# qq456cvb/CPPF2

Measured on AMD Instinct MI355X. Metric: scenes/sec (1/2/4/8 GPU) at 4096 pts x 20k tuples; 5deg5cm match vs ref, higher is better.
Workload: dtype f32

## Files before the change

### cppf2_amd/csrc/cppf_mlp_split.hip

```cpp
#include "cppf_common.h"
#include <atomic>
#include <mutex>
#include <type_traits>

typedef float f32x16 __attribute__((ext_vector_type(16)));
typedef float f32x4 __attribute__((ext_vector_type(4)));
typedef __bf16 bf16x8 __attribute__((ext_vector_type(8)));

__host__ __device__ constexpr int rs_waves(int nt) { return nt >= 6 ? 4 : 8; }
#define RS_RESLAYER 0
#define RS_LINEAR 1
#define RS_SUMGATHER 2
#define RS_ENCODE 3
#define RS_SUMENCODE 5
__host__ __device__ constexpr int rs_waves_mode(int nt, int mode) { return mode == RS_LINEAR ? 8 : rs_waves(nt); }
__host__ __device__ constexpr int rs_stage_tiles(int mode) { return 16; }
__host__ __device__ constexpr int rs_wgs_per_cu(int mode) { return 1; }
#define RS_FRAG_BYTES 1024
__host__ __device__ constexpr int rs_stage_bytes(int stg) { return stg * 3 * RS_FRAG_BYTES; }
__host__ __device__ constexpr int rs_tile_bytes(int pc) { return pc * RS_FRAG_BYTES; }

#ifndef RS_DEEP_PREFETCH
#define RS_DEEP_PREFETCH 0
#endif
// ... 325 lines not shown
};

template <int NT, int PC>
__device__ __forceinline__ void rs_decode_epilogue(f32x16 (&o)[NT], const RsDecode& dc, int64_t row, bool in, int g, float bs) {
  static_assert(NT == 6, "6 coordinates x 32 bins");
  if (PC == 2) {
#pragma unroll
    for (int u = 0; u < 6; ++u) o[u] *= bs;
  }
  if (dc.prior) {
    const float* pr = dc.prior + row * 192 + 4 * g;
#pragma unroll
    for (int u = 0; u < 6; ++u) {
#pragma unroll
      for (int q = 0; q < 4; ++q) {
        const f32x4 v = *reinterpret_cast<const f32x4*>(pr + 32 * u + 8 * q);
        o[u][4 * q + 0] += v.x; o[u][4 * q + 1] += v.y; o[u][4 * q + 2] += v.z; o[u][4 * q + 3] += v.w;
      }
    }
  } else if (dc.prior_pos) {
    const float* pp = dc.prior_pos + row * 6;
    const float is = dc.prior_inv_sigma;
#pragma unroll
    for (int u = 0; u < 6; ++u) {
      const float pos = pp[u];
#pragma unroll
      for (int e = 0; e < 16; ++e) {
        const float z = ((float)((e & 3) + 8 * (e >> 2) + 4 * g) - pos) * is;
        o[u][e] += (z * z) * -0.5f;
      }
    }
  }
  float back[6], tot[6];
#pragma unroll
  for (int u = 0; u < 6; ++u) {
    float m = o[u][0];
#pragma unroll
    for (int e = 1; e < 16; ++e) m = fmaxf(m, o[u][e]);
    m = fmaxf(m, __shfl_xor(m, 32));
#pragma unroll
    for (int e = 0; e < 16; ++e) o[u][e] = softmax_exp(o[u][e] - m);
    back[u] = 0.0f;
  }
#pragma unroll
  for (int q = 0; q < 4; ++q) {
    float ta[6][4], tb[6][4], fwd[6];
#pragma unroll
    for (int u = 0; u < 6; ++u) {
      ta[u][0] = back[u] + o[u][4 * q + 0];
      ta[u][1] = ta[u][0] + o[u][4 * q + 1];
      ta[u][2] = ta[u][1] + o[u][4 * q + 2];
      ta[u][3] = ta[u][2] + o[u][4 * q + 3];
    }
#pragma unroll
    for (int u = 0; u < 6; ++u) fwd[u] = __shfl_xor(ta[u][3], 32);
#pragma unroll
    for (int u = 0; u < 6; ++u) {
      tb[u][0] = fwd[u] + o[u][4 * q + 0];
      tb[u][1] = tb[u][0] + o[u][4 * q + 1];
      tb[u][2] = tb[u][1] + o[u][4 * q + 2];
      tb[u][3] = tb[u][2] + o[u][4 * q + 3];
    }
#pragma unroll
    for (int u = 0; u < 6; ++u) {
      back[u] = __shfl_xor(tb[u][3], 32);
      tot[u] = g ? tb[u][3] : back[u];
#pragma unroll
      for (int i = 0; i < 4; ++i) o[u][4 * q + i] = g ? tb[u][i] : ta[u][i];
    }
  }
  const float* ur = dc.uniforms + row * 6;
#pragma unroll
  for (int u = 0; u < 6; ++u) {
    const float target = ur[u] * tot[u];
    int cnt = 0;
#pragma unroll
    for (int e = 0; e < 16; ++e) cnt += (o[u][e] <= target) ? 1 : 0;
    cnt += __shfl_xor(cnt, 32);
    if (in && g == 0) dc.bins[row * 6 + u] = cnt < 31 ? cnt : 31;
  }
}

__device__ __forceinline__ void rs_claim_store(int* p, int v) { __hip_atomic_store(p, v, __ATOMIC_RELAXED, __HIP_MEMORY_SCOPE_WORKGROUP); }
__device__ __forceinline__ int rs_claim_load(int* p) { return __hip_atomic_load(p, __ATOMIC_RELAXED, __HIP_MEMORY_SCOPE_WORKGROUP); }

struct RsTap {
  float* out = nullptr;
  int64_t ld = 0;
};

struct RsGather {
  const int32_t* gidx = nullptr;
  const float* table = nullptr;
  int slots = 0, head = 0, fshift = 0;
  int64_t tld = 0;
  const float* pts = nullptr;
  const float* nrm = nullptr;
  const int32_t* pt_off = nullptr;
  const int32_t* tup_off = nullptr;
  int B = 0;
  int* sched = nullptr;
};

struct RsRow3 {
  float x, y, z;
};

__device__ __forceinline__ void rs_encode_tiles(char* slots, int lane, int g, const float* __restrict__ pts, const float* __restrict__ nrm,
                                                const float* __restrict__ table, int fshift, int g0, int g1, int g2, int g3, int g4) {
  constexpr int PI_[10] = {0, 0, 0, 0, 1, 1, 1, 2, 2, 3}, PJ_[10] = {1, 2, 3, 4, 2, 3, 4, 3, 4, 4};
  const int gi[5] = {g0, g1, g2, g3, g4};
  float v[48];
  {
    float p[5][3];
#pragma unroll
    for (int q = 0; q < 5; ++q) {
      const RsRow3 r = *reinterpret_cast<const RsRow3*>(pts + 3 * (int64_t)gi[q]);
      p[q][0] = r.x; p[q][1] = r.y; p[q][2] = r.z;
    }
#pragma unroll
    for (int q = 0; q < 10; ++q)
#pragma unroll
      for (int c = 0; c < 3; ++c) v[3 * q + c] = p[PI_[q]][c] - p[PJ_[q]][c];
  }
  {
    float n[5][3];
#pragma unroll
    for (int q = 0; q < 5; ++q) {
      const RsRow3 r = *reinterpret_cast<const RsRow3*>(nrm + 3 * (int64_t)gi[q]);
      n[q][0] = r.x; n[q][1] = r.y; n[q][2] = r.z;
    }
#pragma unroll
    for (int q = 0; q < 10; ++q) {
      const float* ni = n[PI_[q]];
      const float* nj = n[PJ_[q]];
      const float s_ = (ni[0] * nj[0] + ni[1] * nj[1]) + ni[2] * nj[2];
      v[30 + q] = fmaxf(s_, -s_);
    }
  }
  {
    const float* d0 = table + ((int64_t)g0 << fshift);
    const f32x4 a = *reinterpret_cast<const f32x4*>(d0), b = *reinterpret_cast<const f32x4*>(d0 + 4);
    v[40] = a.x; v[41] = a.y; v[42] = a.z; v[43] = a.w; v[44] = b.x; v[45] = b.y; v[46] = b.z; v[47] = b.w;
  }
#pragma unroll
  for (int s = 0; s < 3; ++s) {
    f32x4 lo, hi;
    lo.x = g ? v[16 * s + 8] : v[16 * s + 0]; lo.y = g ? v[16 * s + 9] : v[16 * s + 1];
    lo.z = g ? v[16 * s + 10] : v[16 * s + 2]; lo.w = g ? v[16 * s + 11] : v[16 * s + 3];
    hi.x = g ? v[16 * s + 12] : v[16 * s + 4]; hi.y = g ? v[16 * s + 13] : v[16 * s + 5];
    hi.z = g ? v[16 * s + 14] : v[16 * s + 6]; hi.w = g ? v[16 * s + 15] : v[16 * s + 7];
    *reinterpret_cast<f32x4*>(slots + s * 2048 + lane * 16) = lo;
    *reinterpret_cast<f32x4*>(slots + s * 2048 + 1024 + lane * 16) = hi;
  }
}

__device__ __forceinline__ void rs_encode_coord_tiles(char* slots, int lane, int g, const float* __restrict__ pts, int g0, int g1, int g2,
                                                      int g3, int g4) {
  constexpr int PI_[10] = {0, 0, 0, 0, 1, 1, 1, 2, 2, 3}, PJ_[10] = {1, 2, 3, 4, 2, 3, 4, 3, 4, 4};
  const int gi[5] = {g0, g1, g2, g3, g4};
  float p[5][3], v[32];
#pragma unroll
  for (int q = 0; q < 5; ++q) {
    const RsRow3 r = *reinterpret_cast<const RsRow3*>(pts + 3 * (int64_t)gi[q]);
    p[q][0] = r.x; p[q][1] = r.y; p[q][2] = r.z;
  }
#pragma unroll
  for (int q = 0; q < 10; ++q)
#pragma unroll
    for (int c = 0; c < 3; ++c) v[3 * q + c] = p[PI_[q]][c] - p[PJ_[q]][c];
  v[30] = 0.0f; v[31] = 0.0f;
#pragma unroll
  for (int s = 0; s < 2; ++s) {
    f32x4 lo, hi;
    lo.x = g ? v[16 * s + 8] : v[16 * s + 0]; lo.y = g ? v[16 * s + 9] : v[16 * s + 1];
    lo.z = g ? v[16 * s + 10] : v[16 * s + 2]; lo.w = g ? v[16 * s + 11] : v[16 * s + 3];
    hi.x = g ? v[16 * s + 12] : v[16 * s + 4]; hi.y = g ? v[16 * s + 13] : v[16 * s + 5];
    hi.z = g ? v[16 * s + 14] : v[16 * s + 6]; hi.w = g ? v[16 * s + 15] : v[16 * s + 7];
    *reinterpret_cast<f32x4*>(slots + s * 2048 + lane * 16) = lo;
    *reinterpret_cast<f32x4*>(slots + s * 2048 + 1024 + lane * 16) = hi;
  }
}

template <int NT, bool PROJ, bool GATHER, bool DECODE = false, int PC = 3, int MODE = RS_RESLAYER>
__global__ __launch_bounds__(64 * rs_waves_mode(NT, MODE), rs_wgs_per_cu(MODE)) void reslayer_split_kernel(const float* x, int64_t ldx, int k_in, float* out,
                                                                              int64_t ldo, int64_t rows,
                                                                              const char* __restrict__ wq,
                                                                              const float* __restrict__ b1,
                                                                              const float* __restrict__ b0, int chain,
                                                                              RsGather ga, RsDecode dc, RsTap tap, float wscale) {
  const float bs = (PC == 2) ? 1.0f / wscale : 1.0f;
  constexpr int WAVES = rs_waves_mode(NT, MODE), THREADS = 64 * WAVES, BLOCK_ROWS = 32 * WAVES;
  constexpr int T0 = PROJ ? 2 * NT : NT;
  constexpr bool LIN = MODE == RS_LINEAR;
  static_assert(!LIN || (!PROJ && !GATHER && !DECODE), "a plain Linear has one product");
  constexpr bool SUMG = MODE == RS_SUMGATHER || MODE == RS_SUMENCODE;
  constexpr bool LOCAL_IDX = MODE == RS_ENCODE || MODE == RS_SUMENCODE;
  static_assert(!SUMG || (PROJ && !GATHER), "the table sums stand for columns of a projection layer's input");
  static_assert(MODE != RS_ENCODE || (GATHER && !DECODE), "RS_ENCODE is a form of the gathering launch");
  constexpr bool PF = RS_DEEP_PREFETCH && WAVES == 4;
  extern __shared__ __attribute__((aligned(16))) char s_ring[];
  const int lane = threadIdx.x & 63;
  const int wave = __builtin_amdgcn_readfirstlane(threadIdx.x >> 6);
  const int r = lane & 31, g = lane >> 5;
  const int ks1 = (k_in + 15) >> 4;
  const int64_t nblocks = (rows + BLOCK_ROWS - 1) / BLOCK_ROWS;
  int64_t bfirst = blockIdx.x, bstride = gridDim.x, bend = nblocks;
  if (RS_XCD_BLOCKS && (gridDim.x & 7) == 0 && nblocks >= 64) {
    const int64_t xcd = blockIdx.x & 7;
    bfirst = nblocks * xcd / 8 + (blockIdx.x >> 3);
    bend = nblocks * (xcd + 1) / 8;
    bstride = gridDim.x >> 3;
  }
  int* const sched = ga.sched;
  const bool dyn = sched != nullptr && !LIN;
  int* const s_claim = reinterpret_cast<int*>(s_ring + 2 * rs_stage_bytes(rs_stage_tiles(MODE)) + WAVES * 3 * 2048 + (2 + chain) * 32 * NT * 4);
  if (dyn) { bfirst = blockIdx.x; bstride = 0; bend = nblocks; }
  const int64_t mine = dyn ? (bfirst < bend ? 1 : 0) : (bend > bfirst ? (bend - bfirst + bstride - 1) / bstride : 0);
  if (dyn && threadIdx.x == 0) rs_claim_store(&s_claim[0], (int)gridDim.x + atomicAdd(&sched[0], 1));

  constexpr int STG = rs_stage_tiles(MODE), RING_BYTES = 2 * rs_stage_bytes(STG);
  RsStream<NT, T0, WAVES, PC, LIN, STG> ws;
  const int64_t seg_bytes = (int64_t)ks1 * T0 * rs_tile_bytes(PC);
  if (LIN) {
    wq += (int64_t)blockIdx.y * chain * seg_bytes;
    b1 = b1 ? b1 + (int64_t)blockIdx.y * chain * 32 * NT : b1;
    out += (int64_t)blockIdx.y * chain * 32 * NT;
  }
  ws.base = wq;
  ws.ring = s_ring;
  ws.ks1 = ks1;
  ws.seg = 0;
  ws.pos = 0;
  ws.off = 0;
  ws.shape(chain);
  ws.left = mine * ws.chunks;
  ws.stage = 0;
  ws.wave = wave;
  ws.lane = lane;
  ws.prime();
  float* s_b1 = reinterpret_cast<float*>(s_ring + RING_BYTES + WAVES * 3 * 2048);
  float* s_b0 = s_b1 + 32 * NT;
  if (LIN) {
    for (int i = threadIdx.x; i < 32 * NT * chain; i += THREADS) s_b1[i] = b1 ? b1[i] : 0.0f;
  } else {
    for (int i = threadIdx.x; i < 32 * NT; i += THREADS) {
      s_b1[i] = b1[i];
      if (PROJ) s_b0[i] = b0[i];
    }
    for (int i = threadIdx.x; i < 32 * NT * chain; i += THREADS) s_b1[2 * 32 * NT + i] = b1[32 * NT + i];
  }
  __syncthreads();

  RsX<GATHER> xs;
  xs.slots = s_ring + RING_BYTES + wave * (3 * 2048);
  xs.k_in = k_in;
  xs.g = g;
  xs.lane = lane;
  xs.table = ga.table;
  xs.head = ga.head;
  xs.fshift = ga.fshift;
  auto row_of = [&](int64_t blk) {
    const int64_t row = blk * BLOCK_ROWS + wave * 32 + r;
    const int64_t rc = row < rows ? row : rows - 1;
    RsRow rw;
    rw.xrow = LOCAL_IDX ? ga.table : x + rc * ldx;
    rw.g0 = rw.g1 = rw.g2 = rw.g3 = rw.g4 = rw.g5 = rw.g6 = rw.g7 = 0;
    if (GATHER || SUMG) {
      const int32_t* p = ga.gidx + rc * ga.slots;
      int p0 = 0;
      if (LOCAL_IDX) {
        int lo = 0, hi = ga.B;
        while (hi - lo > 1) {
          const int mid = (lo + hi) >> 1;
          if ((int64_t)ga.tup_off[mid] <= rc) lo = mid; else hi = mid;
        }
        p0 = ga.pt_off[lo];
      }
      rw.g0 = p[0];
      rw.g1 = ga.slots > 1 ? p[1] : 0; rw.g2 = ga.slots > 2 ? p[2] : 0; rw.g3 = ga.slots > 3 ? p[3] : 0;
      rw.g4 = ga.slots > 4 ? p[4] : 0; rw.g5 = ga.slots > 5 ? p[5] : 0; rw.g6 = ga.slots > 6 ? p[6] : 0;
      rw.g7 = ga.slots > 7 ? p[7] : 0;
      if (LOCAL_IDX) {
        rw.g0 += p0; rw.g1 += ga.slots > 1 ? p0 : 0; rw.g2 += ga.slots > 2 ? p0 : 0; rw.g3 += ga.slots > 3 ? p0 : 0;
        rw.g4 += ga.slots > 4 ? p0 : 0; rw.g5 += ga.slots > 5 ? p0 : 0; rw.g6 += ga.slots > 6 ? p0 : 0; rw.g7 += ga.slots > 7 ? p0 : 0;
      }
    }
    return rw;
  };
  int64_t next_blk = dyn ? (int64_t)rs_claim_load(&s_claim[0]) : bfirst + bstride;
  int par = 1;
  RsRow cur = row_of(bfirst < bend ? bfirst : 0);
  auto first_tiles = [&](const RsRow rw) {
    if constexpr (MODE == RS_ENCODE) {
      rs_encode_tiles(xs.slots, lane, g, ga.pts, ga.nrm, ga.table, ga.fshift, rw.g0, rw.g1, rw.g2, rw.g3, rw.g4);
    } else if constexpr (MODE == RS_SUMENCODE) {
      rs_encode_coord_tiles(xs.slots, lane, g, ga.pts, rw.g0, rw.g1, rw.g2, rw.g3, rw.g4);
    } else {
      xs.issue(0, 0, rw);
      xs.issue(1, 1, rw);
      xs.issue(2, 2, rw);
    }
  };
  if (bfirst < bend) first_tiles(cur);
  if constexpr (LIN) {
    for (int64_t blk = bfirst; blk < bend; blk += bstride) {
      const int64_t row = blk * BLOCK_ROWS + wave * 32 + r;
      const bool in = row < rows;
      const bool more = blk + bstride < bend;
      const RsRow nxt = row_of(more ? blk + bstride : blk);
#pragma unroll 1
      for (int grp = 0; grp < chain; ++grp) {
        f32x16 acc[NT];
#pragma unroll
        for (int u = 0; u < NT; ++u) rs_load_tile(acc[u], s_b1 + 32 * (grp * NT + u), g);
        rs_product_x<NT, false, PC>(acc, xs, cur, ks1, ws);
        const bool last = grp + 1 == chain;
        if (!last || more) {
          const RsRow nx = last ? nxt : cur;
          xs.issue(0, 0, nx);
          xs.issue(1, 1, nx);
          xs.issue(2, 2, nx);
        }
        if (in) {
          float* orow = out + row * ldo + (int64_t)grp * 32 * NT + 4 * g;
#pragma unroll
          for (int u = 0; u < NT; ++u) {
#pragma unroll
            for (int q = 0; q < 4; ++q) {
              f32x4 v;
              v.x = acc[u][4 * q + 0]; v.y = acc[u][4 * q + 1]; v.z = acc[u][4 * q + 2]; v.w = acc[u][4 * q + 3];
              if (PC == 2) v *= bs;
              *reinterpret_cast<f32x4*>(orow + 32 * u + 8 * q) = v;
            }
          }
        }
      }
      cur = nxt;
    }
    RS_WAIT(0, 15);
    return;
  }
  for (int64_t blk = bfirst; blk < bend;) {
    const int64_t row = blk * BLOCK_ROWS + wave * 32 + r;
    const bool in = row < rows;
    const float* xrow = cur.xrow;
    const int64_t nb = dyn ? next_blk : blk + bstride;
    const bool more = nb < bend;
    if (dyn && more) ws.left += ws.chunks;
    const RsRow nxt = row_of(more ? nb : blk);
    int claim = 0;
    if (dyn && threadIdx.x == 0) claim = atomicAdd(&sched[0], 1);
    f32x16 acc[2 * NT];
    f32x16 (&h)[NT] = *reinterpret_cast<f32x16 (*)[NT]>(&acc[0]);
    f32x16 (&o)[NT] = *reinterpret_cast<f32x16 (*)[NT]>(&acc[NT]);
#pragma unroll
    for (int u = 0; u < T0; ++u) rs_load_tile(acc[u], s_b1 + 32 * u, g);
    if constexpr (SUMG) {
#pragma unroll 1
      for (int i = 0; i < ((RS_DBG & 64) ? 0 : ga.slots); ++i) {
        int p = cur.g0;
        p = i == 1 ? cur.g1 : p; p = i == 2 ? cur.g2 : p; p = i == 3 ? cur.g3 : p; p = i == 4 ? cur.g4 : p;
        p = i == 5 ? cur.g5 : p; p = i == 6 ? cur.g6 : p; p = i == 7 ? cur.g7 : p;
        if (RS_DBG & 128) p &= 255;
        const float* trow = ga.table + ((int64_t)p * ga.tld + (int64_t)i * (32 * T0)) + 4 * g;
#pragma unroll
        for (int u0 = 0; u0 < T0; u0 += 4) {
          f32x4 t[16];
#pragma unroll
          for (int j = 0; j < 16; ++j) t[j] = *reinterpret_cast<const f32x4*>(trow + 32 * (u0 + (j >> 2)) + 8 * (j & 3));
#pragma unroll
          for (int j = 0; j < 16; ++j) {
            f32x16& a = acc[u0 + (j >> 2)];
            const int q = j & 3;
            if (PC == 2) {
              a[4 * q + 0] += t[j].x * wscale; a[4 * q + 1] += t[j].y * wscale; a[4 * q + 2] += t[j].z * wscale; a[4 * q + 3] += t[j].w * wscale;
            } else {
              a[4 * q + 0] += t[j].x; a[4 * q + 1] += t[j].y; a[4 * q + 2] += t[j].z; a[4 * q + 3] += t[j].w;
            }
          }
        }
      }
    }
    if (!PROJ && (WAVES == 8 || RS_EARLY_RESIDUAL)) {
#pragma unroll
      for (int u = 0; u < NT; ++u) {
        if (PC == 2) rs_load_tile_scaled(o[u], ((RS_DBG & 32) ? (const float*)s_b1 : xrow) + 32 * u, g, wscale);
        else rs_load_tile(o[u], ((RS_DBG & 32) ? (const float*)s_b1 : xrow) + 32 * u, g);
      }
    }
    {
      f32x16 (&first)[T0] = *reinterpret_cast<f32x16 (*)[T0]>(&acc[0]);
      rs_product_x<T0, PF, PC>(first, xs, cur, ks1, ws);
    }
#pragma unroll
    for (int u = 0; u < NT; ++u) {
#pragma unroll
      for (int e = 0; e < 16; ++e) h[u][e] = (h[u][e] < 0.0f) ? 0.0f : h[u][e];
    }
    if (!PROJ && WAVES == 4 && !RS_EARLY_RESIDUAL) {
      if (PC == 2) {
#pragma unroll
        for (int u = 0; u < NT; u += 2) {
          rs_load_tile_scaled(o[u], ((RS_DBG & 32) ? (const float*)s_b1 : xrow) + 32 * u, g, wscale);
          if (u + 1 < NT) rs_load_tile_scaled(o[u + 1], ((RS_DBG & 32) ? (const float*)s_b1 : xrow) + 32 * (u + 1), g, wscale);
#pragma unroll
          for (int e = 0; e < 16; ++e) {
            asm volatile("" : "+a"(o[u][e]));
            if (u + 1 < NT) asm volatile("" : "+a"(o[u + 1][e]));
          }
          __builtin_amdgcn_sched_barrier(0);
        }
      } else {
#pragma unroll
        for (int u = 0; u < NT; ++u) rs_load_tile(o[u], ((RS_DBG & 32) ? (const float*)s_b1 : xrow) + 32 * u, g);
      }
    }
    if (dyn && threadIdx.x == 0) rs_claim_store(&s_claim[par], (int)gridDim.x + claim);
    if (more) first_tiles(nxt);
    cur = nxt;
    rs_product_h<NT, NT, PF, PC>(o, h, ws, bs);
    if (tap.out && in) {
      float* trow = tap.out + row * tap.ld + 4 * g;
#pragma unroll
      for (int u = 0; u < NT; ++u) {
#pragma unroll
        for (int q = 0; q < 4; ++q) {
          f32x4 v;
          v.x = o[u][4 * q + 0]; v.y = o[u][4 * q + 1]; v.z = o[u][4 * q + 2]; v.w = o[u][4 * q + 3];
          if (PC == 2) v *= bs;
          *reinterpret_cast<f32x4*>(trow + 32 * u + 8 * q) = v;
        }
      }
    }
#pragma unroll 1
    for (int l = 0; l < chain; ++l) {
      const float* bl = s_b1 + 32 * NT * (2 + l);
#pragma unroll
      for (int u = 0; u < NT; ++u) rs_load_tile(h[u], bl + 32 * u, g);
      rs_product_h<NT, NT, PF, PC>(h, o, ws, bs);
#pragma unroll
      for (int u = 0; u < NT; ++u) {
#pragma unroll
        for (int e = 0; e < 16; ++e) h[u][e] = (h[u][e] < 0.0f) ? 0.0f : h[u][e];
      }
      rs_product_h<NT, NT, PF, PC>(o, h, ws, bs);
    }
    if (DECODE) {
      if constexpr (NT == 6) rs_decode_epilogue<NT, PC>(o, dc, in ? row : rows - 1, in, g, bs);
    } else if (in && (!(RS_DBG & 32) || o[0][0] == 1.2345e30f)) {
      float* orow = out + row * ldo + 4 * g;
#pragma unroll
      for (int u = 0; u < NT; ++u) {
#pragma unroll
        for (int q = 0; q < 4; ++q) {
          f32x4 v;
          v.x = o[u][4 * q + 0]; v.y = o[u][4 * q + 1]; v.z = o[u][4 * q + 2]; v.w = o[u][4 * q + 3];
          if (PC == 2) v *= bs;
          *reinterpret_cast<f32x4*>(orow + 32 * u + 8 * q) = v;
        }
      }
    }
    blk = nb;
    if (dyn) {
      next_blk = rs_claim_load(&s_claim[par]);
      par ^= 1;
    }
  }
  RS_WAIT(0, 15);
  if (dyn && threadIdx.x == 0) {
    if (atomicAdd(&sched[1], 1) == (int)gridDim.x - 1) {
      __hip_atomic_store(&sched[0], 0, __ATOMIC_RELAXED, __HIP_MEMORY_SCOPE_AGENT);
      __hip_atomic_store(&sched[1], 0, __ATOMIC_RELAXED, __HIP_MEMORY_SCOPE_AGENT);
    }
  }
}

static int64_t rs_stream_bytes(int32_t k_in, int32_t n_out, int32_t proj, int32_t chain, int pc) {
  if (k_in <= 0 || !(n_out == 64 || n_out == 128 || n_out == 192 || n_out == 256) || chain < 0 || chain > 15) return -1;
  const int64_t nt = n_out / 32, ks1 = (k_in + 15) / 16;
  return (ks1 * (proj ? 2 : 1) + (1 + 2 * (int64_t)chain) * 2 * nt) * nt * rs_tile_bytes(pc);
}

extern "C" int64_t cppf_reslayer_split_stream_bytes(int32_t k_in, int32_t n_out, int32_t proj, int32_t chain) {
  return rs_stream_bytes(k_in, n_out, proj, chain, 3);
}

static std::atomic<int> g_rs_debug_cus{0};
extern "C" int cppf_reslayer_split_debug_grid(int32_t workgroups) {
  g_rs_debug_cus.store(workgroups > 0 ? workgroups : 0);
  return CPPF_OK;
}

static std::atomic<int> g_rs_reserved_cus{0};
extern "C" int cppf_mlp_reserve_cus(int32_t cus) {
  CPPF_CHECK_ARG(cus <= 1024);
  return cus < 0 ? g_rs_reserved_cus.load() : g_rs_reserved_cus.exchange(cus);
}

template <int NT, bool PROJ, bool GATHER = false, bool DECODE = false, int PC = 3, int MODE = RS_RESLAYER>
static int rs_launch(const float* x, int64_t ldx, int k_in, float* out, int64_t ldo, int64_t rows, const char* wq,
                     const float* b1, const float* b0, int chain, int cus, hipStream_t stream, RsGather ga = RsGather(),
                     RsDecode dc = RsDecode(), RsTap tap = RsTap(), float wscale = 1.0f) {
  constexpr int WAVES = rs_waves_mode(NT, MODE), THREADS = 64 * WAVES, BLOCK_ROWS = 32 * WAVES;
  const int64_t nblocks = (rows + BLOCK_ROWS - 1) / BLOCK_ROWS;
  const int forced = g_rs_debug_cus.load();
  if (forced > 0) cus = forced;
  else cus = cus - g_rs_reserved_cus.load() > cus / 2 ? cus - g_rs_reserved_cus.load() : (cus + 1) / 2;
  cus *= rs_wgs_per_cu(MODE);
  const unsigned grid = (unsigned)(nblocks < cus ? nblocks : cus);
  unsigned gy = 1;
  if (MODE == RS_LINEAR && (int64_t)grid * 2 <= cus) {
    for (int d = chain; d >= 1; --d)
      if (chain % d == 0 && (int64_t)grid * d <= cus) { gy = (unsigned)d; break; }
    chain /= (int)gy;
  }
  const int lds_bytes = 2 * rs_stage_bytes(rs_stage_tiles(MODE)) + WAVES * 3 * 2048 + (MODE == RS_LINEAR ? chain : 2 + chain) * 32 * NT * 4 + 16;
  if (lds_bytes > 160 * 1024 / rs_wgs_per_cu(MODE)) {
    snprintf(g_cppf_err, sizeof(g_cppf_err), "reslayer_split: %d bytes of LDS for the biases of this launch (too many column groups)", lds_bytes);
    return CPPF_EINVAL;
  }
  {
    static std::mutex mu;
    static bool done[64] = {false};
    int dev = 0;
    CPPF_HIP(hipGetDevice(&dev));
    std::lock_guard<std::mutex> lock(mu);
    if (!done[dev & 63]) {
      CPPF_HIP(hipFuncSetAttribute((const void*)reslayer_split_kernel<NT, PROJ, GATHER, DECODE, PC, MODE>,
                                   hipFuncAttributeMaxDynamicSharedMemorySize, 160 * 1024));
      done[dev & 63] = true;
    }
  }
  hipLaunchKernelGGL((reslayer_split_kernel<NT, PROJ, GATHER, DECODE, PC, MODE>), dim3(grid, gy), dim3(THREADS), lds_bytes, stream, x,
                     ldx, k_in, out, ldo, rows, wq, b1, b0, chain, ga, dc, tap, wscale);
  CPPF_LAUNCH_CHECK();
  return CPPF_OK;
}

static int rs_cus() {
  int dev = 0, n_cu = 0;
  if (hipGetDevice(&dev) != hipSuccess || hipDeviceGetAttribute(&n_cu, hipDeviceAttributeMultiprocessorCount, dev) != hipSuccess) return 256;
  return n_cu > 0 ? n_cu : 256;
}

static int rs_dispatch(const float* x, int64_t ldx, int32_t k_in, float* out, int64_t ldo, int32_t n_out, int64_t rows,
                       const void* wq, int64_t wq_bytes, const float* b1, const float* b0, int32_t chain, RsTap tap,
                       int32_t* sched, void* stream, const char* fn) {
  if (!(x && out && wq && b1 && rows >= 0) || !(k_in > 0 && (k_in & 7) == 0 && ldx >= k_in && (ldx & 3) == 0 && (ldo & 3) == 0 && ldo >= n_out) ||
      !(n_out == 64 || n_out == 128 || n_out == 192 || n_out == 256) || !(b0 != nullptr || k_in == n_out) ||
      !(chain >= 0 && chain <= 15) || (((uintptr_t)x | (uintptr_t)out | (uintptr_t)wq | (uintptr_t)tap.out) & 15) != 0 ||
      (tap.out && ((tap.ld & 3) != 0 || tap.ld < n_out)) ||
      wq_bytes != cppf_reslayer_split_stream_bytes(k_in, n_out, b0 != nullptr, chain)) {
    snprintf(g_cppf_err, sizeof(g_cppf_err), "%s: invalid argument (pointers, 16-byte alignment, k_in %% 8, strides %% 4, n_out in "
             "{64,128,192,256}, chain <= 15, stream size)", fn);
    return CPPF_EINVAL;
  }
  if (rows == 0) return CPPF_OK;
  static std::mutex mu;
  static int cus[64] = {0};
  int dev = 0;
  CPPF_HIP(hipGetDevice(&dev));
  {
    std::lock_guard<std::mutex> lock(mu);
    if (cus[dev & 63] == 0) {
      hipDeviceProp_t prop;
      CPPF_HIP(hipGetDeviceProperties(&prop, dev));
      cus[dev & 63] = prop.multiProcessorCount > 0 ? prop.multiProcessorCount : 256;
    }
  }
  const int n_cu = cus[dev & 63];
  const char* w = static_cast<const char*>(wq);
  hipStream_t st = (hipStream_t)stream;
  const bool proj = b0 != nullptr;
  RsGather ga;
  ga.sched = sched;
  const RsDecode dc = RsDecode();
  switch (n_out / 32) {
    case 2: return proj ? rs_launch<2, true>(x, ldx, k_in, out, ldo, rows, w, b1, b0, chain, n_cu, st, ga, dc, tap)
                        : rs_launch<2, false>(x, ldx, k_in, out, ldo, rows, w, b1, b0, chain, n_cu, st, ga, dc, tap);
    case 4: return proj ? rs_launch<4, true>(x, ldx, k_in, out, ldo, rows, w, b1, b0, chain, n_cu, st, ga, dc, tap)
                        : rs_launch<4, false>(x, ldx, k_in, out, ldo, rows, w, b1, b0, chain, n_cu, st, ga, dc, tap);
    case 6: return proj ? rs_launch<6, true>(x, ldx, k_in, out, ldo, rows, w, b1, b0, chain, n_cu, st, ga, dc, tap)
                        : rs_launch<6, false>(x, ldx, k_in, out, ldo, rows, w, b1, b0, chain, n_cu, st, ga, dc, tap);
    default: return proj ? rs_launch<8, true>(x, ldx, k_in, out, ldo, rows, w, b1, b0, chain, n_cu, st, ga, dc, tap)
                         : rs_launch<8, false>(x, ldx, k_in, out, ldo, rows, w, b1, b0, chain, n_cu, st, ga, dc, tap);
  }
}

extern "C" int cppf_reslayer_split(const float* x, int64_t ldx, int32_t k_in, float* out, int64_t ldo, int32_t n_out,
                                   int64_t rows, const void* wq, int64_t wq_bytes, const float* b1, const float* b0,
                                   int32_t chain, int32_t* sched, void* stream) {
  return rs_dispatch(x, ldx, k_in, out, ldo, n_out, rows, wq, wq_bytes, b1, b0, chain, RsTap(), sched, stream, __func__);
}

extern "C" int cppf_reslayer_split_tap(const float* x, int64_t ldx, int32_t k_in, float* first_out, int64_t ld_first, float* out,
                                       int64_t ldo, int32_t n_out, int64_t rows, const void* wq, int64_t wq_bytes,
                                       const float* b1, const float* b0, int32_t chain, int32_t* sched, void* stream) {
  if (!first_out || first_out == out || first_out == x) {
    snprintf(g_cppf_err, sizeof(g_cppf_err), "%s: first_out must be a buffer of its own", __func__);
    return CPPF_EINVAL;
  }
  RsTap tap;
  tap.out = first_out;
  tap.ld = ld_first;
  return rs_dispatch(x, ldx, k_in, out, ldo, n_out, rows, wq, wq_bytes, b1, b0, chain, tap, sched, stream, __func__);
}

extern "C" int cppf_reslayer_split_gather(const float* heads, int64_t ld_heads, int32_t head_cols, const int32_t* gidx,
                                          int32_t slots, const float* table, int32_t fdim, float* out, int64_t ldo,
                                          int32_t n_out, int64_t rows, const void* wq, int64_t wq_bytes, const float* b1,
                                          const float* b0, int32_t chain, int32_t* sched, void* stream) {
  CPPF_CHECK_ARG(heads && gidx && table && out && wq && b1 && b0 && rows >= 0);
  CPPF_CHECK_ARG(head_cols >= 0 && (head_cols & 7) == 0 && ld_heads >= head_cols && (ld_heads & 3) == 0);
  CPPF_CHECK_ARG(slots >= 1 && slots <= 8 && fdim >= 8 && (fdim & (fdim - 1)) == 0);
  CPPF_CHECK_ARG((ldo & 3) == 0 && ldo >= n_out && chain >= 0 && chain <= 15);
  CPPF_CHECK_ARG((((uintptr_t)heads | (uintptr_t)table | (uintptr_t)out | (uintptr_t)wq) & 15) == 0);
  const int k_in = head_cols + slots * fdim;
  CPPF_CHECK_ARG(wq_bytes == cppf_reslayer_split_stream_bytes(k_in, n_out, 1, chain));
  if (n_out != 128) {
    snprintf(g_cppf_err, sizeof(g_cppf_err), "cppf_reslayer_split_gather: n_out = %d (only the 128-wide projection layer of the "
             "tuple encoder has a gathering kernel)", n_out);
    return CPPF_EUNSUPPORTED;
  }
  if (rows == 0) return CPPF_OK;
  int dev = 0, n_cu = 0;
  CPPF_HIP(hipGetDevice(&dev));
  CPPF_HIP(hipDeviceGetAttribute(&n_cu, hipDeviceAttributeMultiprocessorCount, dev));
  RsGather ga;
  ga.gidx = gidx;
  ga.table = table;
  ga.slots = slots;
  ga.head = head_cols;
  ga.fshift = __builtin_ctz((unsigned)fdim);
  ga.sched = sched;
  return rs_launch<4, true, true>(heads, ld_heads, k_in, out, ldo, rows, static_cast<const char*>(wq), b1, b0, chain,
                                  n_cu > 0 ? n_cu : 256, (hipStream_t)stream, ga);
}

extern "C" int cppf_reslayer_split_encode(int B, const float* pts, const float* normals, const int32_t* idx, int32_t k,
                                          const int32_t* pt_off, const int32_t* tup_off, const float* table, int32_t fdim,
                                          float* out, int64_t ldo, int32_t n_out, int64_t rows, const void* wq, int64_t wq_bytes,
                                          const float* b1, const float* b0, int32_t chain, int32_t* sched, void* stream) {
  CPPF_CHECK_ARG(B > 0 && pts && normals && idx && pt_off && tup_off && table && out && wq && b1 && b0 && rows >= 0);
  CPPF_CHECK_ARG(fdim >= 8 && (fdim & (fdim - 1)) == 0 && (ldo & 3) == 0 && ldo >= n_out && chain >= 0 && chain <= 15);
  CPPF_CHECK_ARG((((uintptr_t)table | (uintptr_t)out | (uintptr_t)wq) & 15) == 0);
  if (k != 5 || n_out != 128) {
    snprintf(g_cppf_err, sizeof(g_cppf_err), "cppf_reslayer_split_encode: k = %d, n_out = %d (the kernel builds the 40 pair features of "
             "5-point tuples for the 128-wide projection layer of the tuple encoder)", k, n_out);
    return CPPF_EUNSUPPORTED;
  }
  const int k_in = 40 + k * fdim;
  CPPF_CHECK_ARG(wq_bytes == cppf_reslayer_split_stream_bytes(k_in, n_out, 1, chain));
  if (rows == 0) return CPPF_OK;
  RsGather ga;
  ga.gidx = idx;
  ga.table = table;
  ga.slots = k;
  ga.head = 40;
  ga.fshift = __builtin_ctz((unsigned)fdim);
  ga.pts = pts;
  ga.nrm = normals;
  ga.pt_off = pt_off;
  ga.tup_off = tup_off;
  ga.B = B;
  ga.sched = sched;
  return rs_launch<4, true, true, false, 3, RS_ENCODE>(nullptr, 0, k_in, out, ldo, rows, static_cast<const char*>(wq), b1, b0, chain,
                                                       rs_cus(), (hipStream_t)stream, ga);
}

extern "C" int cppf_reslayer_split_decode_prior(const float* x, int64_t ldx, int32_t k_in, int64_t rows, const void* wq, int64_t wq_bytes,
                                                const float* b1, const float* b0, const float* logit_prior, const float* prior_pos,
                                                float prior_inv_sigma, const float* uniforms, int32_t* bins, int32_t* sched,
                                                void* stream) {
  CPPF_CHECK_ARG(x && wq && b1 && b0 && uniforms && bins && rows >= 0);
  CPPF_CHECK_ARG(!(logit_prior && prior_pos) && (!prior_pos || (prior_inv_sigma > 0.0f && prior_inv_sigma < INFINITY)));
  CPPF_CHECK_ARG(k_in > 0 && (k_in & 7) == 0 && ldx >= k_in && (ldx & 3) == 0);
  CPPF_CHECK_ARG((((uintptr_t)x | (uintptr_t)wq | (uintptr_t)logit_prior) & 15) == 0);
  CPPF_CHECK_ARG(wq_bytes == cppf_reslayer_split_stream_bytes(k_in, 192, 1, 0));
  if (rows == 0) return CPPF_OK;
  int dev = 0, n_cu = 0;
  CPPF_HIP(hipGetDevice(&dev));
  CPPF_HIP(hipDeviceGetAttribute(&n_cu, hipDeviceAttributeMultiprocessorCount, dev));
  RsDecode dc;
  dc.prior = logit_prior;
  dc.prior_pos = prior_pos;
  dc.prior_inv_sigma = prior_pos ? prior_inv_sigma : 0.0f;
  dc.uniforms = uniforms;
  dc.bins = bins;
  RsGather ga;
  ga.sched = sched;
  return rs_launch<6, true, false, true>(x, ldx, k_in, nullptr, 192, rows, static_cast<const char*>(wq), b1, b0, 0,
                                         n_cu > 0 ? n_cu : 256, (hipStream_t)stream, ga, dc);
}


extern "C" int cppf_reslayer_split_decode(const float* x, int64_t ldx, int32_t k_in, int64_t rows, const void* wq, int64_t wq_bytes,
                                          const float* b1, const float* b0, const float* uniforms, int32_t* bins, int32_t* sched,
                                          void* stream) {
  return cppf_reslayer_split_decode_prior(x, ldx, k_in, rows, wq, wq_bytes, b1, b0, nullptr, nullptr, 0.0f, uniforms, bins, sched, stream);
}


extern "C" int64_t cppf_linear_split_stream_bytes(int32_t k_in, int32_t n_out) {
  if (k_in <= 0 || n_out <= 0 || (n_out & 255) != 0) return -1;
  return (int64_t)((k_in + 15) / 16) * (n_out / 32) * rs_tile_bytes(3);
}

extern "C" int cppf_linear_split(const float* x, int64_t ldx, int32_t k_in, float* out, int64_t ldo, int32_t n_out, int64_t rows,
                                 const void* wq, int64_t wq_bytes, const float* bias, void* stream) {
  CPPF_CHECK_ARG(x && out && wq && rows >= 0);
  CPPF_CHECK_ARG(k_in > 0 && (k_in & 7) == 0 && ldx >= k_in && (ldx & 3) == 0 && n_out > 0 && (n_out & 255) == 0 && ldo >= n_out && (ldo & 3) == 0);
  CPPF_CHECK_ARG((((uintptr_t)x | (uintptr_t)out | (uintptr_t)wq) & 15) == 0);
  CPPF_CHECK_ARG(wq_bytes == cppf_linear_split_stream_bytes(k_in, n_out));
  if (rows == 0) return CPPF_OK;
  return rs_launch<8, false, false, false, 3, RS_LINEAR>(x, ldx, k_in, out, ldo, rows, static_cast<const char*>(wq), bias, nullptr,
                                                         n_out / 256, rs_cus(), (hipStream_t)stream);
}

extern "C" int cppf_reslayer_split_sumgather(const float* heads, int64_t ld_heads, int32_t head_cols, const int32_t* gidx,
                                             int32_t slots, const float* tables, int64_t ld_tables, float* out, int64_t ldo,
                                             int32_t n_out, int64_t rows, const void* wq, int64_t wq_bytes, const float* b1,
// ... 155 lines not shown
```

Baseline: 6026.

## Coalesce SUMGATHER table gathers through LDS transpose and defer X tile issue

In the SUMGATHER path, each lane no longer reads scattered 16-byte pieces of its own row's table entry. Gather indices are now broadcast with ds_bpermute so each group of 8 lanes reads one contiguous 128-byte row segment. The data is staged through the X-slot LDS region and re-read in the accumulator layout. Because that LDS region is reused as scratch, the X tile prefetch for SUMGATHER moves to after the gather, which loses the overlap with the previous block's work. It also adds LDS write/read traffic and possible bank conflicts, and may need barriers that the code does not show.

```diff
diff --git a/cppf2_amd/csrc/cppf_mlp_split.hip b/cppf2_amd/csrc/cppf_mlp_split.hip
--- a/cppf2_amd/csrc/cppf_mlp_split.hip
+++ b/cppf2_amd/csrc/cppf_mlp_split.hip
@@ -651,7 +651,8 @@
       xs.issue(2, 2, rw);
     }
   };
-  if (bfirst < bend) first_tiles(cur);
+  constexpr bool LATE_X = SUMG;
+  if (bfirst < bend && !LATE_X) first_tiles(cur);
   if constexpr (LIN) {
     for (int64_t blk = bfirst; blk < bend; blk += bstride) {
       const int64_t row = blk * BLOCK_ROWS + wave * 32 + r;
@@ -712,25 +713,38 @@
         p = i == 1 ? cur.g1 : p; p = i == 2 ? cur.g2 : p; p = i == 3 ? cur.g3 : p; p = i == 4 ? cur.g4 : p;
         p = i == 5 ? cur.g5 : p; p = i == 6 ? cur.g6 : p; p = i == 7 ? cur.g7 : p;
         if (RS_DBG & 128) p &= 255;
-        const float* trow = ga.table + ((int64_t)p * ga.tld + (int64_t)i * (32 * T0)) + 4 * g;
-#pragma unroll
-        for (int u0 = 0; u0 < T0; u0 += 4) {
-          f32x4 t[16];
-#pragma unroll
-          for (int j = 0; j < 16; ++j) t[j] = *reinterpret_cast<const f32x4*>(trow + 32 * (u0 + (j >> 2)) + 8 * (j & 3));
-#pragma unroll
-          for (int j = 0; j < 16; ++j) {
-            f32x16& a = acc[u0 + (j >> 2)];
-            const int q = j & 3;
-            if (PC == 2) {
-              a[4 * q + 0] += t[j].x * wscale; a[4 * q + 1] += t[j].y * wscale; a[4 * q + 2] += t[j].z * wscale; a[4 * q + 3] += t[j].w * wscale;
-            } else {
-              a[4 * q + 0] += t[j].x; a[4 * q + 1] += t[j].y; a[4 * q + 2] += t[j].z; a[4 * q + 3] += t[j].w;
+        const int lr = lane >> 3, lc = lane & 7;
+        const float* const src = ga.table + (int64_t)i * (32 * T0) + 4 * lc;
+        int pk[4];
+#pragma unroll
+        for (int k = 0; k < 4; ++k) pk[k] = __builtin_amdgcn_ds_bpermute((8 * k + lr) << 2, p);
+        float* const img = reinterpret_cast<float*>(xs.slots);
+        constexpr int TG = 2;
+#pragma unroll
+        for (int u0 = 0; u0 < T0; u0 += TG) {
+          f32x4 t[4 * TG];
+#pragma unroll
+          for (int j = 0; j < 4 * TG; ++j)
+            t[j] = *reinterpret_cast<const f32x4*>(src + (int64_t)pk[j & 3] * ga.tld + 32 * (u0 + (j >> 2)));
+#pragma unroll
+          for (int uu = 0; uu < TG; ++uu) {
+#pragma unroll
+            for (int k = 0; k < 4; ++k) *reinterpret_cast<f32x4*>(img + (8 * k + lr) * 36 + 4 * lc) = t[4 * uu + k];
+            f32x16& a = acc[u0 + uu];
+#pragma unroll
+            for (int q = 0; q < 4; ++q) {
+              const f32x4 v = *reinterpret_cast<const f32x4*>(img + r * 36 + 8 * q + 4 * g);
+              if (PC == 2) {
+                a[4 * q + 0] += v.x * wscale; a[4 * q + 1] += v.y * wscale; a[4 * q + 2] += v.z * wscale; a[4 * q + 3] += v.w * wscale;
+              } else {
+                a[4 * q + 0] += v.x; a[4 * q + 1] += v.y; a[4 * q + 2] += v.z; a[4 * q + 3] += v.w;
+              }
             }
           }
         }
       }
     }
+    if constexpr (LATE_X) first_tiles(cur);
     if (!PROJ && (WAVES == 8 || RS_EARLY_RESIDUAL)) {
 #pragma unroll
       for (int u = 0; u < NT; ++u) {
@@ -766,7 +780,7 @@
       }
     }
     if (dyn && threadIdx.x == 0) rs_claim_store(&s_claim[par], (int)gridDim.x + claim);
-    if (more) first_tiles(nxt);
+    if (more && !LATE_X) first_tiles(nxt);
     cur = nxt;
     rs_product_h<NT, NT, PF, PC>(o, h, ws, bs);
     if (tap.out && in) {
```

Measured after the change: 6015, median of 6. Within noise of the previous version (-0.2%).
